# ur-whitelab/hoomd-tf

Hardware: AMD Instinct MI355X
Metric: MD steps/sec + achieved HBM GB/s, 131072 particles NN=128 (131k-particle box of the BASELINE metric) (higher is better)
Workload: dtype f32

## Files before the change

### hoomd_tf_amd/csrc/standin.hip

```cpp
#include <cstdlib>

#include "htf_common.h"
#include "box_math.h"
#include "htf_standin.h"
#include "standin_gate.h"
#include "key_sort.h"

namespace htf {

template <typename T>
__global__ __launch_bounds__(256) void nve_step_kernel(typename Vec4<T>::type *__restrict__ pos,
                                                       typename Vec4<T>::type *__restrict__ vel,
                                                       const typename Vec4<T>::type *__restrict__ force,
                                                       unsigned N, T dt, SBox<T> b) {
    unsigned i = blockIdx.x * blockDim.x + threadIdx.x;
    if (i >= N) return;
    auto p = pos[i];
    auto v = vel[i];
    nve_advance<T>(p, v, force[i], dt, b);
    pos[i] = p;
    vel[i] = v;
}

__device__ __forceinline__ float block_max(float d2, float *s_max) {
    for (int m = 1; m < 64; m <<= 1) d2 = fmaxf(d2, __shfl_xor(d2, m));
    if ((threadIdx.x & 63) == 0) s_max[threadIdx.x >> 6] = d2;
    __syncthreads();
    if (threadIdx.x < 16) {
        d2 = s_max[threadIdx.x];
        for (int m = 1; m < 16; m <<= 1) d2 = fmaxf(d2, __shfl_xor(d2, m));
    }
    return d2;
}

template <typename T>
__device__ __forceinline__ float block_max_disp2(const typename Vec4<T>::type *__restrict__ pos,
                                                 const typename Vec4<T>::type *__restrict__ ref, unsigned N, const SBox<T> &b,
                                                 float *s_max) {
    unsigned i = blockIdx.x * blockDim.x + threadIdx.x;
    float d2 = 0.f;
    if (i < N) d2 = row_disp2<T>(pos[i], ref[i], b);
    return block_max(d2, s_max);
}

__device__ __forceinline__ bool ticket_is_last(float d2, unsigned *__restrict__ work, unsigned *s_last) {
    if (threadIdx.x == 0) {
        unsigned last = 0u;
        if (__float_as_uint(d2) > *(volatile unsigned *)work) atomicMax(work, __float_as_uint(d2));
        __threadfence();
        if (atomicAdd(work + 1, 1u) == gridDim.x - 1u) last = 1u;
        *s_last = last;
    }
    __syncthreads();
    return *s_last != 0u;
}

template <typename T>
__global__ __launch_bounds__(1024) void max_disp_kernel(const typename Vec4<T>::type *__restrict__ pos,
                                                        const typename Vec4<T>::type *__restrict__ ref, unsigned N,
                                                        SBox<T> b, float *__restrict__ out) {
    __shared__ float s_max[16];
    const float d2 = block_max_disp2<T>(pos, ref, N, b, s_max);
    if (threadIdx.x == 0 && __float_as_uint(d2) > *(volatile unsigned *)out)
        atomicMax((unsigned *)out, __float_as_uint(d2));
}

template <typename T, bool CYCLE>
__global__ __launch_bounds__(1024) void check_disp_kernel(const typename Vec4<T>::type *__restrict__ pos,
                                                          const typename Vec4<T>::type *__restrict__ ref, unsigned N,
                                                          SBox<T> b, unsigned *__restrict__ work, float *__restrict__ out,
                                                          float *__restrict__ h_out, htfs_mirror mirror) {
    __shared__ float s_max[16];
    __shared__ unsigned s_last;
    const float d2 = block_max_disp2<T>(pos, ref, N, b, s_max);
    if (!ticket_is_last(d2, work, &s_last)) return;
    if (CYCLE) {
        for (unsigned m = 0; m < mirror.n; ++m) {
            const unsigned *src = (const unsigned *)mirror.src[m];
            unsigned *dst = (unsigned *)mirror.dst[m];
            for (unsigned w = threadIdx.x; w < mirror.words[m]; w += blockDim.x) dst[w] = __builtin_nontemporal_load(src + w);
        }
        __threadfence_system();
        __syncthreads();
    }
    if (threadIdx.x == 0) {
        const float worst = __uint_as_float(atomicExch(work, 0u));
        out[0] = worst;
        work[1] = 0u;
        if (CYCLE) {
            const unsigned cycle = __float_as_uint(out[1]) + 1u;
            out[1] = __uint_as_float(cycle);
            if (h_out != nullptr) {
                h_out[0] = worst;
                __threadfence_system();
                *(volatile unsigned *)(h_out + 1) = cycle;
            }
        }
    }
}

template <typename T>
__global__ __launch_bounds__(1024) void nve_check_kernel(typename Vec4<T>::type *__restrict__ pos, typename Vec4<T>::type *__restrict__ vel,
                                                         const typename Vec4<T>::type *__restrict__ force,
                                                         const typename Vec4<T>::type *__restrict__ ref, unsigned N, T dt, SBox<T> b,
                                                         SBox<T> lb, unsigned *__restrict__ work, float *__restrict__ out) {
    __shared__ float s_max[16];
    __shared__ unsigned s_last;
    unsigned i = blockIdx.x * blockDim.x + threadIdx.x;
    float d2 = 0.f;
    if (i < N) {
        auto p = pos[i];
        auto v = vel[i];
        nve_advance<T>(p, v, force[i], dt, b);
        asm volatile("" : "+v"(p.x), "+v"(p.y), "+v"(p.z));
        pos[i] = p;
        vel[i] = v;
        d2 = row_disp2<T>(p, ref[i], lb);
    }
    d2 = block_max(d2, s_max);
    if (!ticket_is_last(d2, work, &s_last)) return;
    if (threadIdx.x == 0) {
        out[0] = __uint_as_float(atomicExch(work, 0u));
        work[1] = 0u;
    }
}

template <typename T>
__device__ __forceinline__ int cell_coord(T x, T lo, T Linv, int n) {
    int c = (int)floor((x - lo) * Linv * (T)n);
    return c < 0 ? 0 : (c >= n ? n - 1 : c);
}

template <typename T>
__global__ __launch_bounds__(256) void cell_index_kernel(const typename Vec4<T>::type *__restrict__ pos, unsigned Ntot,
                                                         SBox<T> b, int nx, int ny, int nz,
                                                         unsigned *__restrict__ cell_of, Gate gate) {
    if (gate.closed()) return;
    unsigned i = blockIdx.x * blockDim.x + threadIdx.x;
    if (i >= Ntot) return;
    auto p = pos[i];
    if (is_inert(p.x)) {
        cell_of[i] = kDeadCell;
        return;
    }
    int cx = cell_coord<T>(p.x, b.lo[0], b.Linv[0], nx);
    int cy = cell_coord<T>(p.y, b.lo[1], b.Linv[1], ny);
    int cz = cell_coord<T>(p.z, b.lo[2], b.Linv[2], nz);
    cell_of[i] = (unsigned)((cz * ny + cy) * nx + cx);
}

constexpr unsigned kTagSide = 1u << 31;
constexpr unsigned kRangeWrapShift = 28u, kRangeLenMask = (1u << kRangeWrapShift) - 1u;
struct RangesArgs {
    int nx, ny, nz, wx, wy, wz, px, py, pz;
    const unsigned *cell_start;
    uint4 *table;
    unsigned *max_neigh;
};
__device__ __forceinline__ void cell_ranges_body(const unsigned t, const RangesArgs &a) {
    const int nx = a.nx, ny = a.ny, nz = a.nz, wx = a.wx, wy = a.wy, wz = a.wz, px = a.px, py = a.py, pz = a.pz;
    const unsigned *__restrict__ cell_start = a.cell_start;
    uint4 *__restrict__ table = a.table;
    unsigned *__restrict__ max_neigh = a.max_neigh;
    const int nrow = (2 * wy + 1) * (2 * wz + 1);
    if (t == 0) *max_neigh = 0u;
    const unsigned ncell = (unsigned)(nx * ny * nz);
    if (t >= ncell * (unsigned)nrow) return;
    const int c = (int)(t / nrow), r = (int)(t % nrow);
    const int cx = c % nx, cy = (c / nx) % ny, cz = c / (nx * ny);
    const int dz = r / (2 * wy + 1) - wz, dy = r % (2 * wy + 1) - wy;
    int a0 = cx - wx, a1 = cx + wx, b0 = 0, b1 = -1;
    if (a0 < 0) {
        if (px) { b0 = nx + a0; b1 = nx - 1; }
        a0 = 0;
    } else if (a1 >= nx) {
        if (px) { b0 = 0; b1 = a1 - nx; }
        a1 = nx - 1;
    }
    int ay = cy + dy, az = cz + dz;
    bool skip = false;
    unsigned wrap_y = 0u, wrap_z = 0u;
    if (ay < 0) { skip |= !py; ay += ny; wrap_y = 1u; } else if (ay >= ny) { skip |= !py; ay -= ny; wrap_y = 2u; }
    if (az < 0) { skip |= !pz; az += nz; wrap_z = 1u; } else if (az >= nz) { skip |= !pz; az -= nz; wrap_z = 2u; }
    uint4 o = make_uint4(0u, 0u, 0u, 0u);
    if (!skip) {
        const unsigned rowbase = (unsigned)((az * ny + ay) * nx);
        o.x = cell_start[rowbase + a0];
        o.y = (cell_start[rowbase + a1 + 1] - o.x) | (wrap_y << kRangeWrapShift) | (wrap_z << (kRangeWrapShift + 2));
        if (b1 >= b0) {
            o.z = cell_start[rowbase + b0];
            o.w = (cell_start[rowbase + b1 + 1] - o.z) | ((b0 == 0 ? 2u : 1u) << kRangeWrapShift);
        }
    }
    table[t] = o;
}
__global__ __launch_bounds__(256) void cell_ranges_kernel(RangesArgs a, Gate gate) {
    if (gate.closed()) return;
    cell_ranges_body(blockIdx.x * blockDim.x + threadIdx.x, a);
}

template <typename T, int G, bool SHIFT>
__global__ __launch_bounds__(256) void build_nlist_kernel(const typename Vec4<T>::type *__restrict__ pos,
                                                          const typename Vec4<T>::type *__restrict__ pos_sorted,
                                                          unsigned N, SBox<T> b, T rl2, int nx, int ny, int nz,
                                                          int wx, int wy, int wz,
                                                          const unsigned *__restrict__ cell_start, unsigned pitch,
                                                          int type_split,
                                                          unsigned *__restrict__ n_neigh, unsigned *__restrict__ head_list,
                                                          unsigned *__restrict__ nlist, unsigned *__restrict__ max_neigh,
                                                          const uint4 *__restrict__ ranges, Gate gate) {
    if (gate.closed()) return;
    const unsigned lane = threadIdx.x & 63u, g = lane % G, sub = lane / G;
    const unsigned i = ((blockIdx.x * blockDim.x + threadIdx.x) >> 6) * (64 / G) + sub;
    const bool in_range = i < N;
    const auto pi = pos[in_range ? i : 0];
    const bool active = in_range && !is_inert(pi.x);
    const int cx = cell_coord<T>(pi.x, b.lo[0], b.Linv[0], nx);
    const int cy = cell_coord<T>(pi.y, b.lo[1], b.Linv[1], ny);
    const int cz = cell_coord<T>(pi.z, b.lo[2], b.Linv[2], nz);
    const bool side_i = type_split >= 0 && scalar_as_int(pi.w) >= type_split;
    unsigned count = 0;
    unsigned *row = nlist + (size_t)(active ? i : 0) * pitch;
    const int nrow = (2 * wy + 1) * (2 * wz + 1);
    const uint4 *mine = ranges + (size_t)((cz * ny + cy) * nx + cx) * nrow;
    uint4 rg_next = active ? mine[0] : make_uint4(0u, 0u, 0u, 0u);
    for (int r = 0; r < nrow; ++r) {
        const uint4 rg = rg_next;
        if (r + 1 < nrow) rg_next = active ? mine[r + 1] : make_uint4(0u, 0u, 0u, 0u);
        T piy = pi.y, piz = pi.z, six = (T)0;
        if (SHIFT) {
            const unsigned wy_ = (rg.y >> kRangeWrapShift) & 3u, wz_ = rg.y >> (kRangeWrapShift + 2), wx_ = rg.w >> kRangeWrapShift;
            piy += wy_ == 1u ? b.L[1] : (wy_ == 2u ? -b.L[1] : (T)0);
            piz += wz_ == 1u ? b.L[2] : (wz_ == 2u ? -b.L[2] : (T)0);
            six = wx_ == 1u ? b.L[0] : -b.L[0];
        }
#pragma unroll
        for (int part = 0; part < 2; ++part) {
            const unsigned beg = part ? rg.z : rg.x, len = (part ? rg.w : rg.y) & kRangeLenMask;
            const T pix = (SHIFT && part) ? pi.x + six : pi.x;
            const unsigned n = active ? len : 0u;
            for (unsigned t = 0; t < n; t += G) {
                const unsigned m_idx = t + g;
                const auto pk = pos_sorted[beg + min(m_idx, n - 1u)];
                const unsigned tag = (unsigned)scalar_as_int(pk.w);
                const unsigned k = tag & ~kTagSide;
                T ddx = pk.x - pix, ddy = pk.y - piy, ddz = pk.z - piz;
                if (!SHIFT) {
                    ddx = mimg<T>(ddx, b.L[0], b.Linv[0], b.periodic[0]);
                    ddy = mimg<T>(ddy, b.L[1], b.Linv[1], b.periodic[1]);
                    ddz = mimg<T>(ddz, b.L[2], b.Linv[2], b.periodic[2]);
                }
                unsigned long long hits = ballot64(m_idx < n) & ballot64(k != i) & ballot64(ddx * ddx + ddy * ddy + ddz * ddz <= rl2);
                if (type_split >= 0) {
                    asm volatile("" ::: "memory");
                    hits &= ballot64(((tag & kTagSide) != 0u) == side_i);
                }
                const unsigned seg = (unsigned)(hits >> (G * sub)) & (G >= 32 ? ~0u : ((1u << G) - 1u));
                const unsigned rank = count + (unsigned)__popc(seg & ((1u << g) - 1u));
                if (inverse_ballot64(hits) && rank < pitch) row[rank] = k;
                count += (unsigned)__popc(seg);
            }
        }
    }
    if (in_range && g == 0) {
        n_neigh[i] = count < pitch ? count : pitch;
        head_list[i] = i * pitch;
        if (count > *(volatile unsigned *)max_neigh) atomicMax(max_neigh, count);
    }
}


__device__ __forceinline__ void set_tag(float &w, unsigned tag) { w = __uint_as_float(tag); }
__device__ __forceinline__ void set_tag(double &w, unsigned tag) { w = __longlong_as_double((long long)tag); }
__device__ __forceinline__ float bcast_lane_t(float v, unsigned lane) {
    return __int_as_float(__builtin_amdgcn_readlane(__float_as_int(v), (int)lane));
}
__device__ __forceinline__ double bcast_lane_t(double v, unsigned lane) {
    const long long q = __double_as_longlong(v);
    const unsigned lo = (unsigned)__builtin_amdgcn_readlane((int)(unsigned)q, (int)lane);
    const unsigned hi = (unsigned)__builtin_amdgcn_readlane((int)(unsigned)(q >> 32), (int)lane);
    return __longlong_as_double((long long)(((unsigned long long)hi << 32) | lo));
}
__device__ __forceinline__ unsigned bperm_u(unsigned lane_idx, unsigned v) {
    return (unsigned)__builtin_amdgcn_ds_bpermute((int)(lane_idx << 2), (int)v);
}
__device__ __forceinline__ float bperm_t(unsigned lane_idx, float v) { return __uint_as_float(bperm_u(lane_idx, __float_as_uint(v))); }
__device__ __forceinline__ double bperm_t(unsigned lane_idx, double v) {
    const unsigned long long q = (unsigned long long)__double_as_longlong(v);
    const unsigned lo = bperm_u(lane_idx, (unsigned)q), hi = bperm_u(lane_idx, (unsigned)(q >> 32));
    return __longlong_as_double((long long)(((unsigned long long)hi << 32) | lo));
}
constexpr int kCellBatch = 8;

template <typename T, bool SHIFT>
__global__ __launch_bounds__(256) void build_nlist_cells_kernel(const typename Vec4<T>::type *__restrict__ pos_sorted, unsigned N,
                                                                SBox<T> b, T rl2, unsigned ncell, int nrow,
                                                                const unsigned *__restrict__ cell_start, unsigned pitch,
                                                                int type_split, unsigned *__restrict__ n_neigh,
                                                                unsigned *__restrict__ head_list, unsigned *__restrict__ nlist,
                                                                unsigned *__restrict__ max_neigh,
                                                                const uint4 *__restrict__ ranges, unsigned split, Gate gate) {
    if (gate.closed()) return;
    using V4 = typename Vec4<T>::type;
    const unsigned lane = threadIdx.x & 63u;
    const unsigned wv = __builtin_amdgcn_readfirstlane((blockIdx.x * blockDim.x + threadIdx.x) >> 6);
    const unsigned c = wv / split, b0 = wv % split;
    if (c >= ncell) return;
    const unsigned p_begin = cell_start[c], p_end = cell_start[c + 1];
    if (p_begin + b0 * (unsigned)kCellBatch >= p_end) return;
    if (p_end - p_begin <= 64u) {
        const bool local = lane < p_end - p_begin && ((unsigned)scalar_as_int(pos_sorted[p_begin + lane].w) & ~kTagSide) < N;
        if (ballot64(local) == 0ull) return;
    }

    unsigned beg = 0u, len = 0u;
    T shx = (T)0, shy = (T)0, shz = (T)0;
    if (lane < 2u * (unsigned)nrow) {
        const uint4 rg = ranges[(size_t)c * nrow + (lane >> 1)];
        const bool wrapped = (lane & 1u) != 0u;
        beg = wrapped ? rg.z : rg.x;
        len = (wrapped ? rg.w : rg.y) & kRangeLenMask;
        if (SHIFT) {
            const unsigned wy_ = (rg.y >> kRangeWrapShift) & 3u, wz_ = rg.y >> (kRangeWrapShift + 2), wx_ = rg.w >> kRangeWrapShift;
            shy = wy_ == 1u ? b.L[1] : (wy_ == 2u ? -b.L[1] : (T)0);
            shz = wz_ == 1u ? b.L[2] : (wz_ == 2u ? -b.L[2] : (T)0);
            shx = !wrapped ? (T)0 : (wx_ == 1u ? b.L[0] : -b.L[0]);
        }
    }
    unsigned incl = len;
#pragma unroll
    for (unsigned d = 1; d < 64u; d <<= 1) {
        const unsigned up = bperm_u(lane >= d ? lane - d : lane, incl);
        incl += lane >= d ? up : 0u;
    }
    const unsigned start = incl - len;
    const unsigned total = (unsigned)__builtin_amdgcn_readlane((int)incl, 63);
    const bool any_shift = SHIFT && ballot64(len != 0u && (shx != (T)0 || shy != (T)0 || shz != (T)0)) != 0ull;

    for (unsigned pb = p_begin + b0 * (unsigned)kCellBatch; pb < p_end; pb += split * (unsigned)kCellBatch) {
        const unsigned np = min(p_end - pb, (unsigned)kCellBatch);
        V4 me;
        me.x = me.y = me.z = (T)0;
        set_tag(me.w, ~0u);
        if (lane < np) me = pos_sorted[pb + lane];
        const unsigned my_tag = (unsigned)scalar_as_int(me.w);
        if (ballot64(lane < np && (my_tag & ~kTagSide) < N) == 0ull) continue;
        unsigned tag_p[kCellBatch], count[kCellBatch];
        T px[kCellBatch], py[kCellBatch], pz[kCellBatch];
        unsigned row_p[kCellBatch];
#pragma unroll
        for (int p = 0; p < kCellBatch; ++p) {
            tag_p[p] = ~0u;
            px[p] = py[p] = pz[p] = (T)0;
            count[p] = 0u;
            row_p[p] = 0u;
            if ((unsigned)p < np) {
                tag_p[p] = (unsigned)__builtin_amdgcn_readlane((int)my_tag, p);
                px[p] = in_vgpr(bcast_lane_t(me.x, p));
                py[p] = in_vgpr(bcast_lane_t(me.y, p));
                pz[p] = in_vgpr(bcast_lane_t(me.z, p));
                row_p[p] = (tag_p[p] & ~kTagSide) * pitch;
            }
        }
        for (unsigned q0 = 0; q0 < total; q0 += 64u) {
            const unsigned q = q0 + lane;
            unsigned at = 0u;
#pragma unroll
            for (unsigned step = 32u; step != 0u; step >>= 1) {
                const unsigned t = at + step;
                at = bperm_u(t, start) <= q ? t : at;
            }
            const bool valid = q < total;
            const unsigned src = bperm_u(at, beg) + (q - bperm_u(at, start));
            V4 pk;
            pk.x = pk.y = pk.z = (T)0;
            set_tag(pk.w, ~0u);
            if (valid) pk = pos_sorted[src];
            if (any_shift) {
                pk.x -= bperm_t(at, shx);
                pk.y -= bperm_t(at, shy);
                pk.z -= bperm_t(at, shz);
            }
            const unsigned tag = (unsigned)scalar_as_int(pk.w);
            const unsigned k = tag & ~kTagSide;
            const unsigned long long vmask = ballot64(valid);
#pragma unroll
            for (int p = 0; p < kCellBatch; ++p) {
                const unsigned i = tag_p[p] & ~kTagSide;
                if (i >= N) continue;
                T ddx = pk.x - px[p], ddy = pk.y - py[p], ddz = pk.z - pz[p];
                if (!SHIFT) {
                    ddx = mimg<T>(ddx, b.L[0], b.Linv[0], b.periodic[0]);
                    ddy = mimg<T>(ddy, b.L[1], b.Linv[1], b.periodic[1]);
                    ddz = mimg<T>(ddz, b.L[2], b.Linv[2], b.periodic[2]);
                }
                unsigned long long hits = vmask & ballot64(k != i) & ballot64(ddx * ddx + ddy * ddy + ddz * ddz <= rl2);
                if (type_split >= 0) {
                    asm volatile("" ::: "memory");
                    hits &= ballot64(((tag ^ tag_p[p]) & kTagSide) == 0u);
                }
                const unsigned rank = __builtin_amdgcn_mbcnt_hi((unsigned)(hits >> 32), __builtin_amdgcn_mbcnt_lo((unsigned)hits, count[p]));
                if (inverse_ballot64(hits) && rank < pitch) nlist[row_p[p] + rank] = k;
                count[p] += (unsigned)__builtin_popcountll(hits);
            }
        }
        unsigned cnt = 0u;
#pragma unroll
        for (int p = 0; p < kCellBatch; ++p) cnt = lane == (unsigned)p ? count[p] : cnt;
        if (lane < np) {
            const unsigned i = my_tag & ~kTagSide;
            if (i < N) {
                n_neigh[i] = cnt < pitch ? cnt : pitch;
                head_list[i] = i * pitch;
                if (cnt > *(volatile unsigned *)max_neigh) atomicMax(max_neigh, cnt);
            }
        }
    }
}

}

using namespace htf;

extern "C" int htfs_nve_step(void *d_pos, void *d_vel, const void *d_force, int dtype, unsigned N, double dt,
                             const htf_box *box, htf_stream stream) {
    HTF_REQUIRE(d_pos && d_vel && d_force && box, "htfs_nve_step: null pointer");
    if (N == 0) return HTF_OK;
    unsigned grid = (N + 255) / 256;
    if (dtype == HTF_F32)
        hipLaunchKernelGGL((nve_step_kernel<float>), dim3(grid), dim3(256), 0, (hipStream_t)stream, (float4 *)d_pos, (float4 *)d_vel, (const float4 *)d_force, N, (float)dt, make_sbox<float>(box));
    else
        hipLaunchKernelGGL((nve_step_kernel<double>), dim3(grid), dim3(256), 0, (hipStream_t)stream, (double4 *)d_pos, (double4 *)d_vel, (const double4 *)d_force, N, dt, make_sbox<double>(box));
    return check_launch("nve_step_kernel");
}

extern "C" int htfs_nve_step_check(void *d_pos, void *d_vel, const void *d_force, int dtype, unsigned N, double dt, const htf_box *box,
                                   const htfs_nlist *nl, float *d_disp2, htf_stream stream) {
    HTF_REQUIRE(d_pos && d_vel && d_force && box && nl && d_disp2, "htfs_nve_step_check: null pointer");
    HTF_REQUIRE(nl->ref && nl->scratch, "htfs_nve_step_check: the list has no reference positions or no scratch");
    HTF_REQUIRE(dtype == HTF_F32 || dtype == HTF_F64, "htfs_nve_step_check: bad dtype %d", dtype);
    if (N == 0) return HTF_OK;
    const unsigned ncell = (unsigned)(nl->ncell3[0] * nl->ncell3[1] * nl->ncell3[2]);
    HTF_REQUIRE(ncell > 0, "htfs_nve_step_check: no cells");
    unsigned *work = nl->scratch + HTFS_SCRATCH_WORK(ncell);
    const unsigned grid = (N + 1023) / 1024;
    if (dtype == HTF_F32)
        hipLaunchKernelGGL((nve_check_kernel<float>), dim3(grid), dim3(1024), 0, (hipStream_t)stream, (float4 *)d_pos, (float4 *)d_vel, (const float4 *)d_force, (const float4 *)nl->ref, N, (float)dt, make_sbox<float>(box), make_sbox<float>(&nl->box), work, d_disp2);
    else
        hipLaunchKernelGGL((nve_check_kernel<double>), dim3(grid), dim3(1024), 0, (hipStream_t)stream, (double4 *)d_pos, (double4 *)d_vel, (const double4 *)d_force, (const double4 *)nl->ref, N, dt, make_sbox<double>(box), make_sbox<double>(&nl->box), work, d_disp2);
    return check_launch("nve_check_kernel");
}

extern "C" int htfs_max_displacement2(const void *d_pos, const void *d_ref, int dtype, unsigned N, const htf_box *box,
                                      float *d_out, htf_stream stream) {
    HTF_REQUIRE(d_pos && d_ref && box && d_out, "htfs_max_displacement2: null pointer");
    if (N == 0) return HTF_OK;
    unsigned grid = (N + 1023) / 1024;
    if (dtype == HTF_F32)
        hipLaunchKernelGGL((max_disp_kernel<float>), dim3(grid), dim3(1024), 0, (hipStream_t)stream, (const float4 *)d_pos, (const float4 *)d_ref, N, make_sbox<float>(box), d_out);
    else
        hipLaunchKernelGGL((max_disp_kernel<double>), dim3(grid), dim3(1024), 0, (hipStream_t)stream, (const double4 *)d_pos, (const double4 *)d_ref, N, make_sbox<double>(box), d_out);
    return check_launch("max_disp_kernel");
}

extern "C" int htfs_check_displacement2(const void *d_pos, const void *d_ref, int dtype, unsigned N, const htf_box *box,
                                        unsigned *d_work, float *d_out, float *h_out, const htfs_mirror *mirror, htf_stream stream) {
    using namespace htf;
    HTF_REQUIRE(d_pos && d_ref && box && d_work && d_out, "htfs_check_displacement2: null pointer");
    HTF_REQUIRE(N > 0, "htfs_check_displacement2: no rows");
    htfs_mirror mr = {};
    if (mirror != nullptr) {
        mr = *mirror;
        HTF_REQUIRE(mr.n <= HTFS_MIRROR_MAX, "htfs_check_displacement2: %u mirrors (at most %d)", mr.n, HTFS_MIRROR_MAX);
        for (unsigned m = 0; m < mr.n; ++m)
            HTF_REQUIRE(mr.src[m] && mr.dst[m] && ((uintptr_t)mr.src[m] & 3) == 0 && ((uintptr_t)mr.dst[m] & 3) == 0,
                        "htfs_check_displacement2: mirror %u: null or unaligned pointer", m);
    }
    unsigned grid = (N + 1023) / 1024;
    if (dtype == HTF_F32)
        hipLaunchKernelGGL((check_disp_kernel<float, true>), dim3(grid), dim3(1024), 0, (hipStream_t)stream, (const float4 *)d_pos, (const float4 *)d_ref, N, make_sbox<float>(box), d_work, d_out, h_out, mr);
    else
        hipLaunchKernelGGL((check_disp_kernel<double, true>), dim3(grid), dim3(1024), 0, (hipStream_t)stream, (const double4 *)d_pos, (const double4 *)d_ref, N, make_sbox<double>(box), d_work, d_out, h_out, mr);
    return check_launch("check_disp_kernel");
}

namespace htf {
struct Reimage {
    double L[3], c[3];
};
template <typename T>
__device__ __forceinline__ T reimage1(T x, double L, double c) {
    return L > 0.0 ? (T)((double)x - L * rint(((double)x - c) / L)) : x;
}

template <typename V>
__global__ __launch_bounds__(256) void bins_finish_kernel(RangesArgs ra, unsigned nb_ranges, V *__restrict__ dest, const V *__restrict__ src,
                                                          const unsigned *__restrict__ stage, const unsigned *__restrict__ cell_of,
                                                          unsigned *__restrict__ order, unsigned *__restrict__ count, unsigned n,
                                                          int type_split, V *__restrict__ ref, unsigned n_ref,
                                                          unsigned *__restrict__ counter, Reimage im, Gate gate) {
    if (gate.closed()) return;
    if (blockIdx.x < nb_ranges) {
        const unsigned t = blockIdx.x * blockDim.x + threadIdx.x;
        if (count != nullptr && t < (unsigned)(ra.nx * ra.ny * ra.nz)) count[t] = 0u;
        cell_ranges_body(t, ra);
        return;
    }
    const unsigned i = (blockIdx.x - nb_ranges) * blockDim.x + threadIdx.x;
    if (i == 0 && counter != nullptr) *counter += 1u;
    if (i >= n || i >= ra.cell_start[ra.nx * ra.ny * ra.nz]) return;
    const unsigned k = stage[i];
    V p = src[k];
    const unsigned c = cell_of[k];
    const unsigned cb = ra.cell_start[c], ce = ra.cell_start[c + 1];
    unsigned slot = cb;
    for (unsigned j = cb; j < ce; ++j) slot += stage[j] < k ? 1u : 0u;
    order[slot] = k;
    if (ref != nullptr && k < n_ref) ref[k] = p;
    p.x = reimage1(p.x, im.L[0], im.c[0]);
    p.y = reimage1(p.y, im.L[1], im.c[1]);
    p.z = reimage1(p.z, im.L[2], im.c[2]);
    set_tag(p.w, k | ((type_split >= 0 && scalar_as_int(p.w) >= type_split) ? kTagSide : 0u));
    dest[slot] = p;
}

template <typename T>
__global__ __launch_bounds__(256) void cell_index_count_kernel(const typename Vec4<T>::type *__restrict__ pos, unsigned Ntot, SBox<T> b,
                                                               int nx, int ny, int nz, unsigned *__restrict__ cell_of,
                                                               unsigned *__restrict__ count, Reimage im, Gate gate) {
    if (gate.closed()) return;
    unsigned i = blockIdx.x * blockDim.x + threadIdx.x;
    if (i >= Ntot) return;
    auto p = pos[i];
    if (is_inert(p.x)) {
        cell_of[i] = kDeadCell;
        return;
    }
    int cx = cell_coord<T>(reimage1(p.x, im.L[0], im.c[0]), b.lo[0], b.Linv[0], nx);
    int cy = cell_coord<T>(reimage1(p.y, im.L[1], im.c[1]), b.lo[1], b.Linv[1], ny);
    int cz = cell_coord<T>(reimage1(p.z, im.L[2], im.c[2]), b.lo[2], b.Linv[2], nz);
    const unsigned c = (unsigned)((cz * ny + cy) * nx + cx);
    cell_of[i] = c;
    atomicAdd(&count[c], 1u);
}

template <typename V, bool TAG>
__global__ void gather4_kernel(V *__restrict__ dest, const V *__restrict__ src, const int *__restrict__ order, unsigned n,
                               int type_split, Gate gate, const unsigned *__restrict__ n_live = nullptr) {
    if (gate.closed()) return;
    const unsigned i = blockIdx.x * blockDim.x + threadIdx.x;
    if (i >= n) return;
    if (n_live != nullptr && i >= *n_live) return;
    const unsigned k = (unsigned)order[i];
    V p = src[k];
    if (TAG) set_tag(p.w, k | ((type_split >= 0 && scalar_as_int(p.w) >= type_split) ? kTagSide : 0u));
    dest[i] = p;
}
}

namespace htf {
__global__ __launch_bounds__(256) void cell_count_kernel(const unsigned *__restrict__ cell_of, unsigned n,
                                                         unsigned *__restrict__ count, Gate gate) {
    if (gate.closed()) return;
    const unsigned i = blockIdx.x * blockDim.x + threadIdx.x;
    if (i < n && cell_of[i] != kDeadCell) atomicAdd(&count[cell_of[i]], 1u);
}

constexpr unsigned kScanThreads = 256, kScanPer = 8, kScanChunk = kScanThreads * kScanPer;
__global__ __launch_bounds__(kScanThreads) void cell_scan_kernel(const unsigned *__restrict__ count, unsigned ncell,
                                                         unsigned *__restrict__ start, unsigned *__restrict__ cursor, Gate gate) {
    if (gate.closed()) return;
    __shared__ unsigned s_wave[kScanThreads / 64], s_carry[kScanThreads / 64];
    const unsigned t = threadIdx.x, lane = t & 63u, wave = t >> 6;
    const unsigned base = blockIdx.x * kScanChunk;
    unsigned before_blk = 0;
    {
        const uint4 *p = reinterpret_cast<const uint4 *>(count);
        for (unsigned i = t; i < base / 4; i += kScanThreads) {
            const uint4 v = p[i];
            before_blk += (v.x + v.y) + (v.z + v.w);
        }
        before_blk = group_sum_u<64>(before_blk);
        if (lane == 0) s_carry[wave] = before_blk;
    }
    const unsigned first = base + t * kScanPer;
    unsigned c[kScanPer];
#pragma unroll
    for (unsigned i = 0; i < kScanPer; ++i) c[i] = first + i < ncell ? count[first + i] : 0u;
    unsigned sum = 0;
#pragma unroll
    for (unsigned i = 0; i < kScanPer; ++i) sum += c[i];
    unsigned incl = sum;
#pragma unroll
    for (unsigned off = 1; off < 64; off <<= 1) {
        const unsigned v = (unsigned)__shfl_up((int)incl, off);
        if (lane >= off) incl += v;
    }
    if (lane == 63) s_wave[wave] = incl;
    __syncthreads();
    unsigned before = 0, total = 0, carry = 0;
#pragma unroll
    for (unsigned w = 0; w < kScanThreads / 64; ++w) {
        const unsigned v = s_wave[w];
        before += w < wave ? v : 0u;
        total += v;
        carry += s_carry[w];
    }
    unsigned run = carry + before + (incl - sum);
#pragma unroll
    for (unsigned i = 0; i < kScanPer; ++i)
        if (first + i < ncell) {
            start[first + i] = run;
            cursor[first + i] = run;
            run += c[i];
        }
    if (blockIdx.x == gridDim.x - 1 && t == 0) start[ncell] = carry + total;
}

__global__ __launch_bounds__(256) void cell_scatter_kernel(const unsigned *__restrict__ cell_of, unsigned n,
                                                           unsigned *__restrict__ cursor, unsigned *__restrict__ order, Gate gate) {
    if (gate.closed()) return;
    const unsigned i = blockIdx.x * blockDim.x + threadIdx.x;
    if (i < n && cell_of[i] != kDeadCell) order[atomicAdd(&cursor[cell_of[i]], 1u)] = i;
}

__global__ __launch_bounds__(256) void cell_order_kernel(const unsigned *__restrict__ start, unsigned ncell,
                                                         unsigned *__restrict__ order, unsigned *__restrict__ count, Gate gate) {
    if (gate.closed()) return;
    const unsigned c = blockIdx.x * blockDim.x + threadIdx.x;
    if (c >= ncell) return;
    count[c] = 0u;
    const unsigned b = start[c], e = start[c + 1];
    for (unsigned i = b + 1; i < e; ++i) {
        const unsigned v = order[i];
        unsigned j = i;
        while (j > b && order[j - 1] > v) {
            order[j] = order[j - 1];
            --j;
        }
        order[j] = v;
    }
}
}

static int zero_counts(unsigned *count, unsigned ncell, hipStream_t s) {
    HTF_REQUIRE(((uintptr_t)count & 15) == 0, "binning scratch must be 16-byte aligned (cell_scan_kernel reads it with 16-byte loads)");
    HTF_CHECK_HIP(hipMemsetAsync(count, 0, (size_t)ncell * sizeof(unsigned), s));
    return HTF_OK;
}
static int zero_nlist_scratch(const htfs_nlist *l, hipStream_t s) {
    const unsigned ncell = (unsigned)(l->ncell3[0] * l->ncell3[1] * l->ncell3[2]);
    HTF_REQUIRE(l->scratch && ncell > 0, "htfs_rebuild_nlist: no scratch, or no cells");
    if (int rc = zero_counts(l->scratch, ncell, s)) return rc;
    HTF_CHECK_HIP(hipMemsetAsync(l->scratch + HTFS_SCRATCH_WORK(ncell), 0, 2 * sizeof(unsigned), s));
    return HTF_OK;
}

extern "C" int htfs_cell_sort(const unsigned *d_cell_of, unsigned Ntot, unsigned ncell, unsigned *d_scratch,
                              unsigned *d_cell_start, unsigned *d_order, htf_stream stream) {
    using namespace htf;
    HTF_REQUIRE(d_cell_of && d_scratch && d_cell_start && d_order, "htfs_cell_sort: null pointer");
    HTF_REQUIRE(ncell > 0, "htfs_cell_sort: no cells");
    hipStream_t s = (hipStream_t)stream;
    unsigned *count = d_scratch, *cursor = d_scratch + ncell;
    if (int rc = zero_counts(count, ncell, s)) return rc;
    if (Ntot) hipLaunchKernelGGL(cell_count_kernel, dim3((Ntot + 255) / 256), dim3(256), 0, s, d_cell_of, Ntot, count, kOpenGate);
    hipLaunchKernelGGL(cell_scan_kernel, dim3((ncell + kScanChunk - 1) / kScanChunk), dim3(kScanThreads), 0, s, count, ncell, d_cell_start, cursor, kOpenGate);
    if (Ntot) hipLaunchKernelGGL(cell_scatter_kernel, dim3((Ntot + 255) / 256), dim3(256), 0, s, d_cell_of, Ntot, cursor, d_order, kOpenGate);
    hipLaunchKernelGGL(cell_order_kernel, dim3((ncell + 255) / 256), dim3(256), 0, s, d_cell_start, ncell, d_order, count, kOpenGate);
    return check_launch("htfs_cell_sort");
}

static int gather4(void *d_dest, const void *d_src, const int *d_order, int dtype, unsigned n, bool tag, int type_split,
                   htf_stream stream, const unsigned *d_n_live = nullptr) {
    using namespace htf;
    HTF_REQUIRE(d_dest && d_src && d_order, "htfs_gather4_tagged: null pointer");
    HTF_REQUIRE(!tag || n <= kTagSide, "htfs_gather4_tagged: %u particles do not fit the 31-bit tag", n);
    if (n == 0) return HTF_OK;
    const dim3 grid((n + 255) / 256), block(256);
    hipStream_t s = (hipStream_t)stream;
    if (dtype == HTF_F32) {
        if (tag) hipLaunchKernelGGL((gather4_kernel<float4, true>), grid, block, 0, s, (float4 *)d_dest, (const float4 *)d_src, d_order, n, type_split, kOpenGate, d_n_live);
        else hipLaunchKernelGGL((gather4_kernel<float4, false>), grid, block, 0, s, (float4 *)d_dest, (const float4 *)d_src, d_order, n, type_split, kOpenGate, d_n_live);
    } else {
        if (tag) hipLaunchKernelGGL((gather4_kernel<double4, true>), grid, block, 0, s, (double4 *)d_dest, (const double4 *)d_src, d_order, n, type_split, kOpenGate, d_n_live);
        else hipLaunchKernelGGL((gather4_kernel<double4, false>), grid, block, 0, s, (double4 *)d_dest, (const double4 *)d_src, d_order, n, type_split, kOpenGate, d_n_live);
    }
    return check_launch("gather4_kernel");
}

extern "C" int htfs_gather4_tagged(void *d_dest, const void *d_src, const int *d_order, int dtype, unsigned n, int type_split,
                                   htf_stream stream) {
    return gather4(d_dest, d_src, d_order, dtype, n, true, type_split, stream);
}

extern "C" int htfs_gather4_tagged_live(void *d_dest, const void *d_src, const int *d_order, int dtype, unsigned n_max,
                                        const unsigned *d_n_live, int type_split, htf_stream stream) {
    HTF_REQUIRE(d_n_live, "htfs_gather4_tagged_live: null pointer");
    return gather4(d_dest, d_src, d_order, dtype, n_max, true, type_split, stream, d_n_live);
}

template <typename T, typename V4>
__global__ __launch_bounds__(256) void slab_classify_kernel(const V4 *__restrict__ pos, unsigned N, const T *__restrict__ bounds,
                                                            int world, int rank, T r_ghost, unsigned *__restrict__ key) {
    const unsigned i = blockIdx.x * blockDim.x + threadIdx.x;
    if (i >= N) return;
    const T x = pos[i].x;
    int owner = 0;
    for (int c = 1; c < world; ++c) owner += (bounds[c] <= x) ? 1 : 0;
    const int left = (rank + world - 1) % world, right = (rank + 1) % world;
    unsigned dest;
    if (world == 2)
        dest = owner != rank ? 2u : 0u;
    else
        dest = owner == rank ? 0u : (owner == left ? 1u : (owner == right ? 2u : 3u));
    const bool near_l = x < bounds[owner] + r_ghost, near_r = x >= bounds[owner + 1] - r_ghost;
    const unsigned cls = near_l ? (near_r ? 2u : 1u) : (near_r ? 3u : 0u);
    key[i] = dest * 4u + cls;
}

extern "C" int htfs_slab_classify(const void *d_pos, int dtype, unsigned N, const void *d_bounds, int world, int rank,
                                  double r_ghost, unsigned *d_key, htf_stream stream) {
    HTF_REQUIRE(d_pos && d_bounds && d_key, "htfs_slab_classify: null pointer");
    HTF_REQUIRE(world >= 2 && rank >= 0 && rank < world, "htfs_slab_classify: rank %d of %d", rank, world);
    if (N == 0) return HTF_OK;
    const unsigned grid = (N + 255) / 256;
    if (dtype == HTF_F32)
        hipLaunchKernelGGL((slab_classify_kernel<float, float4>), dim3(grid), dim3(256), 0, (hipStream_t)stream, (const float4 *)d_pos, N,
                           (const float *)d_bounds, world, rank, (float)r_ghost, d_key);
    else
        hipLaunchKernelGGL((slab_classify_kernel<double, double4>), dim3(grid), dim3(256), 0, (hipStream_t)stream, (const double4 *)d_pos,
                           N, (const double *)d_bounds, world, rank, r_ghost, d_key);
    return check_launch("slab_classify_kernel");
}

extern "C" int htfs_key_sort16(const unsigned *d_key, unsigned N, unsigned *d_scratch, unsigned *d_start, unsigned *d_order,
                               htf_stream stream) {
    HTF_REQUIRE(d_key && d_scratch && d_start && d_order, "htfs_key_sort16: null pointer");
    return htf::key_sort<16>(d_key, N, nullptr, d_scratch, d_start, d_order, (hipStream_t)stream);
}

struct SegTable {
    unsigned n;
    unsigned src[HTFS_MAX_SEGMENTS], dst[HTFS_MAX_SEGMENTS], cnt[HTFS_MAX_SEGMENTS];
};

__global__ __launch_bounds__(256) void segment_copy_kernel(unsigned *__restrict__ dst, const unsigned *__restrict__ src,
                                                           unsigned row_words, SegTable t, unsigned total_rows) {
    const unsigned w = blockIdx.x * blockDim.x + threadIdx.x;
    if (w >= total_rows * row_words) return;
    unsigned row = w / row_words;
    const unsigned col = w - row * row_words;
    unsigned seg = 0;
#pragma unroll 1
    while (seg + 1 < t.n && row >= t.cnt[seg]) {
        row -= t.cnt[seg];
        ++seg;
    }
    dst[(size_t)(t.dst[seg] + row) * row_words + col] = src[(size_t)(t.src[seg] + row) * row_words + col];
}

extern "C" int htfs_segment_copy(void *d_dst, const void *d_src, unsigned row_bytes, unsigned n_segments,
                                 const unsigned *src_start, const unsigned *dst_start, const unsigned *count, htf_stream stream) {
    HTF_REQUIRE(d_dst && d_src && src_start && dst_start && count, "htfs_segment_copy: null pointer");
    HTF_REQUIRE(n_segments >= 1 && n_segments <= HTFS_MAX_SEGMENTS && row_bytes % 4 == 0 && row_bytes > 0,
                "htfs_segment_copy: need 1..%d segments of whole 32-bit words", HTFS_MAX_SEGMENTS);
    SegTable t;
    t.n = 0;
    unsigned total = 0;
    for (unsigned s = 0; s < n_segments; ++s) {
        if (count[s] == 0) continue;
        t.src[t.n] = src_start[s];
        t.dst[t.n] = dst_start[s];
        t.cnt[t.n] = count[s];
        total += count[s];
        ++t.n;
    }
    if (total == 0) return HTF_OK;
    const unsigned words = row_bytes / 4;
    const unsigned grid = (unsigned)(((size_t)total * words + 255) / 256);
    hipLaunchKernelGGL(segment_copy_kernel, dim3(grid), dim3(256), 0, (hipStream_t)stream, (unsigned *)d_dst, (const unsigned *)d_src,
                       words, t, total);
    return check_launch("segment_copy_kernel");
}

extern "C" int htfs_cell_index(const void *d_pos, int dtype, unsigned Ntot, const htf_box *box, const int *ncell3,
                               unsigned *d_cell_of, htf_stream stream) {
    HTF_REQUIRE(d_pos && box && ncell3 && d_cell_of, "htfs_cell_index: null pointer");
    if (Ntot == 0) return HTF_OK;
    unsigned grid = (Ntot + 255) / 256;
    if (dtype == HTF_F32)
        hipLaunchKernelGGL((cell_index_kernel<float>), dim3(grid), dim3(256), 0, (hipStream_t)stream, (const float4 *)d_pos, Ntot, make_sbox<float>(box), ncell3[0], ncell3[1], ncell3[2], d_cell_of, kOpenGate);
    else
        hipLaunchKernelGGL((cell_index_kernel<double>), dim3(grid), dim3(256), 0, (hipStream_t)stream, (const double4 *)d_pos, Ntot, make_sbox<double>(box), ncell3[0], ncell3[1], ncell3[2], d_cell_of, kOpenGate);
    return check_launch("cell_index_kernel");
}

struct FinishArgs {
    unsigned n;
    htf::Reimage im;
    const unsigned *stage;
    unsigned *count;
};

static int build_nlist_impl(const htfs_nlist *l, const void *d_pos, int dtype, unsigned N, htf_stream stream, htf::Gate gate,
                            const FinishArgs *fin) {
    using namespace htf;
    HTF_REQUIRE(l && d_pos && l->pos_sorted && l->cell_start && l->n_neigh && l->head_list && l->nlist && l->max_neigh,
                "htfs_build_nlist: null pointer");
    const htf_box *box = &l->box;
    const int *ncell3 = l->ncell3, *stencil3 = l->stencil3;
    const unsigned *d_cell_start = l->cell_start;
    const void *d_pos_sorted = l->pos_sorted;
    const unsigned pitch = l->pitch;
    const int type_split = l->type_split;
    const double r_list = l->r_list;
    unsigned *d_n_neigh = l->n_neigh, *d_head_list = l->head_list, *d_nlist = l->nlist, *d_max_neigh = l->max_neigh;
    HTF_REQUIRE(pitch > 0, "htfs_build_nlist: pitch must be > 0");
    for (int d = 0; d < 3; ++d) {
        const double w = (box->hi[d] - box->lo[d]) / ncell3[d];
        const int sw = stencil3[d];
        HTF_REQUIRE((sw == 0 && ncell3[d] == 1) || (sw >= 1 && sw <= 2 && ncell3[d] >= 2 * sw + 1 && w * sw >= r_list * (1.0 - 1e-12)),
                    "htfs_build_nlist: along %d need 1 cell, or >= 2w+1 cells with w cells spanning r_list (got %d cells of %g, stencil %d, r_list %g)",
                    d, ncell3[d], w, sw, r_list);
    }
    if (N == 0) return HTF_OK;
    const unsigned ncell = (unsigned)(ncell3[0] * ncell3[1] * ncell3[2]);
    const unsigned nrow = (unsigned)((2 * stencil3[1] + 1) * (2 * stencil3[2] + 1));
    HTF_REQUIRE(l->ranges && ((uintptr_t)l->ranges & 15) == 0, "htfs_build_nlist: ranges must be a 16-byte aligned table of 4 * ncell * rows words");
    uint4 *d_ranges = (uint4 *)l->ranges;
    const RangesArgs ra = {ncell3[0], ncell3[1], ncell3[2], stencil3[0], stencil3[1], stencil3[2], (int)box->periodic[0],
                           (int)box->periodic[1], (int)box->periodic[2], d_cell_start, d_ranges, d_max_neigh};
    const unsigned nb_ranges = (ncell * nrow + 255) / 256;
    if (fin == nullptr) {
        hipLaunchKernelGGL(cell_ranges_kernel, dim3(nb_ranges), dim3(256), 0, (hipStream_t)stream, ra, gate);
    } else {
        const unsigned nb = nb_ranges + (fin->n + 255) / 256 + (fin->n == 0 ? 1u : 0u);
        if (dtype == HTF_F32)
            hipLaunchKernelGGL((bins_finish_kernel<float4>), dim3(nb), dim3(256), 0, (hipStream_t)stream, ra, nb_ranges, (float4 *)l->pos_sorted,
                               (const float4 *)d_pos, fin->stage, l->cell_of, l->order, fin->count, fin->n, type_split, (float4 *)l->ref, N, l->counter, fin->im, gate);
        else
            hipLaunchKernelGGL((bins_finish_kernel<double4>), dim3(nb), dim3(256), 0, (hipStream_t)stream, ra, nb_ranges, (double4 *)l->pos_sorted,
                               (const double4 *)d_pos, fin->stage, l->cell_of, l->order, fin->count, fin->n, type_split, (double4 *)l->ref, N, l->counter, fin->im, gate);
    }
    const bool fine = stencil3[0] == 2 || stencil3[1] == 2 || stencil3[2] == 2;
#define HTFS_NL(T, V4, G)                                                                                              \
    if (shift) HTFS_NL_(T, V4, G, true); else HTFS_NL_(T, V4, G, false)
#define HTFS_NL_(T, V4, G, S)                                                                                          \
    hipLaunchKernelGGL((build_nlist_kernel<T, G, S>), dim3((N + 4 * (64 / G) - 1) / (4 * (64 / G))), dim3(256), 0, (hipStream_t)stream, \
                       (const V4 *)d_pos, (const V4 *)d_pos_sorted, N, make_sbox<T>(box), (T)(r_list * r_list), ncell3[0],  \
                       ncell3[1], ncell3[2], stencil3[0], stencil3[1], stencil3[2], d_cell_start, pitch,      \
                       type_split, d_n_neigh, d_head_list, d_nlist, d_max_neigh, (const uint4 *)d_ranges, gate)
#define HTFS_NLC(T, V4)                                                                                                \
    if (shift) HTFS_NLC_(T, V4, true); else HTFS_NLC_(T, V4, false)
#define HTFS_NLC_(T, V4, S)                                                                                            \
    hipLaunchKernelGGL((build_nlist_cells_kernel<T, S>), dim3((ncell * cell_split + 3) / 4), dim3(256), 0, (hipStream_t)stream, \
                       (const V4 *)d_pos_sorted, N, make_sbox<T>(box), (T)(r_list * r_list), ncell, (int)nrow, d_cell_start, pitch, \
                       type_split, d_n_neigh, d_head_list, d_nlist, d_max_neigh, (const uint4 *)d_ranges, cell_split, gate)
    bool shift = true;
    for (int d = 0; d < 3; ++d) shift = shift && (!box->periodic[d] || ncell3[d] >= 7);
#ifdef HTF_AB_VARIANTS
    static const bool per_particle = std::getenv("HTFS_NLIST_PER_PARTICLE") != nullptr, per_cell = std::getenv("HTFS_NLIST_PER_CELL") != nullptr;
#else
    constexpr bool per_particle = false, per_cell = false;
#endif
    const bool reimaged = fin != nullptr && (fin->im.L[0] > 0.0 || fin->im.L[1] > 0.0 || fin->im.L[2] > 0.0);
    const bool by_cell = per_cell || reimaged || (!per_particle && ncell >= 1024u);
    const unsigned cell_split = ncell <= 12288u ? 2u : 1u;
    if (by_cell) {
        if (dtype == HTF_F32) { HTFS_NLC(float, float4); } else { HTFS_NLC(double, double4); }
    } else if (dtype == HTF_F32) {
        if (fine) { HTFS_NL(float, float4, 8); } else { HTFS_NL(float, float4, 16); }
    } else {
        if (fine) { HTFS_NL(double, double4, 8); } else { HTFS_NL(double, double4, 16); }
    }
#undef HTFS_NL
#undef HTFS_NL_
#undef HTFS_NLC
#undef HTFS_NLC_
    return check_launch("build_nlist_kernel");
}

extern "C" int htfs_build_nlist(const htfs_nlist *nl, const void *d_pos, int dtype, unsigned N, htf_stream stream) {
    return build_nlist_impl(nl, d_pos, dtype, N, stream, htf::kOpenGate, nullptr);
}

static int rebuild_nlist_impl(const htfs_nlist *l, const void *d_pos, int dtype, unsigned N, unsigned Ntot, bool scratch_clean,
                              htf_stream stream, htf::Gate gate) {
    using namespace htf;
    HTF_REQUIRE(l && d_pos && l->cell_of && l->scratch && l->cell_start && l->order && l->pos_sorted, "htfs_rebuild_nlist: null pointer");
    HTF_REQUIRE(Ntot >= N, "htfs_rebuild_nlist: Ntot %u < N %u", Ntot, N);
    if (N == 0) return HTF_OK;
    const htf_box *box = &l->box;
    const int *ncell3 = l->ncell3;
    const unsigned ncell = (unsigned)(ncell3[0] * ncell3[1] * ncell3[2]);
    HTF_REQUIRE(ncell > 0, "htfs_rebuild_nlist: no cells");
    hipStream_t s = (hipStream_t)stream;
    unsigned *count = l->scratch, *cursor = l->scratch + ncell, *stage = l->scratch + HTFS_SCRATCH_STAGE(ncell);
    if (!scratch_clean)
        if (int rc = zero_nlist_scratch(l, s)) return rc;
    const unsigned grid = (Ntot + 255) / 256;
    Reimage im = {};
    for (int d = 0; d < 3; ++d) {
        im.L[d] = !box->periodic[d] ? l->image_L[d] : 0.0;
        im.c[d] = 0.5 * (box->lo[d] + box->hi[d]);
        HTF_REQUIRE(im.L[d] == 0.0 || im.L[d] >= box->hi[d] - box->lo[d], "htfs_rebuild_nlist: image length %g along axis %d is shorter than the grid", im.L[d], d);
    }
    if (dtype == HTF_F32)
        hipLaunchKernelGGL((cell_index_count_kernel<float>), dim3(grid), dim3(256), 0, s, (const float4 *)d_pos, Ntot, make_sbox<float>(box),
                           ncell3[0], ncell3[1], ncell3[2], l->cell_of, count, im, gate);
    else
        hipLaunchKernelGGL((cell_index_count_kernel<double>), dim3(grid), dim3(256), 0, s, (const double4 *)d_pos, Ntot, make_sbox<double>(box),
                           ncell3[0], ncell3[1], ncell3[2], l->cell_of, count, im, gate);
    hipLaunchKernelGGL(cell_scan_kernel, dim3((ncell + kScanChunk - 1) / kScanChunk), dim3(kScanThreads), 0, s, count, ncell, l->cell_start, cursor, gate);
    hipLaunchKernelGGL(cell_scatter_kernel, dim3(grid), dim3(256), 0, s, l->cell_of, Ntot, cursor, stage, gate);
    const FinishArgs fin = {Ntot, im, stage, count};
    return build_nlist_impl(l, d_pos, dtype, N, stream, gate, &fin);
}

extern "C" int htfs_rebuild_nlist(const htfs_nlist *nl, const void *d_pos, int dtype, unsigned N, unsigned Ntot, int scratch_clean,
                                  htf_stream stream) {
    return rebuild_nlist_impl(nl, d_pos, dtype, N, Ntot, scratch_clean != 0, stream, htf::kOpenGate);
}

static int gated_rebuild(const htfs_nlist *nl, const void *d_pos, int dtype, unsigned N, unsigned Ntot, bool scratch_clean, float *d_disp2,
                         double threshold2, unsigned *d_stat2, unsigned *h_stat2, htf_stream stream) {
    htfs_nlist l = *nl;
    l.max_neigh = d_stat2;
    l.counter = d_stat2 + 1;
    int rc = rebuild_nlist_impl(&l, d_pos, dtype, N, Ntot, scratch_clean, stream, htf::Gate{d_disp2, (float)threshold2});
    if (rc != HTF_OK) return rc;
    if (h_stat2 != nullptr)
        HTF_CHECK_HIP(hipMemcpyAsync(h_stat2, d_stat2, 2 * sizeof(unsigned), hipMemcpyDeviceToHost, (hipStream_t)stream));
    return HTF_OK;
}

extern "C" int htfs_check_rebuild_nlist(const htfs_nlist *nl, const void *d_pos, int dtype, unsigned N, unsigned Ntot, int scratch_clean,
                                        float *d_disp2, double threshold2, unsigned *d_stat2, unsigned *h_stat2, htf_stream stream) {
    using namespace htf;
    HTF_REQUIRE(nl && nl->ref && nl->scratch && d_pos && d_disp2 && d_stat2, "htfs_check_rebuild_nlist: null pointer");
    if (N == 0) return HTF_OK;
    const unsigned ncell = (unsigned)(nl->ncell3[0] * nl->ncell3[1] * nl->ncell3[2]);
    HTF_REQUIRE(ncell > 0, "htfs_check_rebuild_nlist: no cells");
    hipStream_t s = (hipStream_t)stream;
    unsigned *work = nl->scratch + HTFS_SCRATCH_WORK(ncell);
    if (!scratch_clean)
        if (int rc = zero_nlist_scratch(nl, s)) return rc;
    const unsigned grid = (N + 1023) / 1024;
    const htfs_mirror none = {};
    if (dtype == HTF_F32)
        hipLaunchKernelGGL((check_disp_kernel<float, false>), dim3(grid), dim3(1024), 0, s, (const float4 *)d_pos, (const float4 *)nl->ref, N, make_sbox<float>(&nl->box), work, d_disp2, (float *)nullptr, none);
    else
        hipLaunchKernelGGL((check_disp_kernel<double, false>), dim3(grid), dim3(1024), 0, s, (const double4 *)d_pos, (const double4 *)nl->ref, N, make_sbox<double>(&nl->box), work, d_disp2, (float *)nullptr, none);
    int rc = check_launch("check_disp_kernel");
    if (rc != HTF_OK) return rc;
    return gated_rebuild(nl, d_pos, dtype, N, Ntot, true, d_disp2, threshold2, d_stat2, h_stat2, stream);
}

extern "C" int htfs_rebuild_nlist_gated(const htfs_nlist *nl, const void *d_pos, int dtype, unsigned N, unsigned Ntot, int scratch_clean,
                                        float *d_disp2, double threshold2, unsigned *d_stat2, unsigned *h_stat2, int h_stat2_by_mail,
                                        htf_stream stream) {
    HTF_REQUIRE(nl && nl->ref && nl->scratch && d_pos && d_disp2 && d_stat2, "htfs_rebuild_nlist_gated: null pointer");
    if (N == 0) return HTF_OK;
    return gated_rebuild(nl, d_pos, dtype, N, Ntot, scratch_clean != 0, d_disp2, threshold2, d_stat2, h_stat2_by_mail ? nullptr : h_stat2,
                         stream);
}
```

Before: 13790.

## Replace per-lane binary search with LDS run-boundary bitmap in cell nlist build

Replaces the six-step ds_bpermute binary search that maps each candidate slot to its source cell range with a per-wave LDS bitmap of run boundaries, using mbcnt to rank and a single permute to find the source offset. It also precomputes row and side masks as scalar ballots, derives self-exclusion from slot index instead of tag compare, and caps SGPRs. The intent is to cut cross-lane permute traffic and VALU work in the inner loop of neighbor-list construction. It adds LDS usage and a fallback path when the candidate total exceeds the bitmap size. The self-exclusion test assumes the i-particle appears at its own sorted index in the candidate stream.

```diff
diff --git a/hoomd_tf_amd/csrc/standin.hip b/hoomd_tf_amd/csrc/standin.hip
--- a/hoomd_tf_amd/csrc/standin.hip
+++ b/hoomd_tf_amd/csrc/standin.hip
@@ -291,15 +291,17 @@
     return __longlong_as_double((long long)(((unsigned long long)hi << 32) | lo));
 }
 constexpr int kCellBatch = 8;
+constexpr unsigned kMapBits = 2048u;
 
 template <typename T, bool SHIFT>
-__global__ __launch_bounds__(256) void build_nlist_cells_kernel(const typename Vec4<T>::type *__restrict__ pos_sorted, unsigned N,
-                                                                SBox<T> b, T rl2, unsigned ncell, int nrow,
-                                                                const unsigned *__restrict__ cell_start, unsigned pitch,
-                                                                int type_split, unsigned *__restrict__ n_neigh,
-                                                                unsigned *__restrict__ head_list, unsigned *__restrict__ nlist,
-                                                                unsigned *__restrict__ max_neigh,
-                                                                const uint4 *__restrict__ ranges, unsigned split, Gate gate) {
+__global__ __launch_bounds__(256) __attribute__((amdgpu_num_sgpr(80)))
+void build_nlist_cells_kernel(const typename Vec4<T>::type *__restrict__ pos_sorted, unsigned N,
+                              SBox<T> b, T rl2, unsigned ncell, int nrow,
+                              const unsigned *__restrict__ cell_start, unsigned pitch,
+                              int type_split, unsigned *__restrict__ n_neigh,
+                              unsigned *__restrict__ head_list, unsigned *__restrict__ nlist,
+                              unsigned *__restrict__ max_neigh,
+                              const uint4 *__restrict__ ranges, unsigned split, Gate gate) {
     if (gate.closed()) return;
     using V4 = typename Vec4<T>::type;
     const unsigned lane = threadIdx.x & 63u;
@@ -337,6 +339,26 @@
     const unsigned total = (unsigned)__builtin_amdgcn_readlane((int)incl, 63);
     const bool any_shift = SHIFT && ballot64(len != 0u && (shx != (T)0 || shy != (T)0 || shz != (T)0)) != 0ull;
 
+    __shared__ unsigned s_map[4 * (kMapBits / 32u)];
+    unsigned *const map = s_map + (threadIdx.x >> 6) * (kMapBits / 32u);
+    const bool mapped = total <= kMapBits;
+    unsigned delta_c = 0u, lane_c = 0u, map_lo = 0u, map_hi = 0u;
+    if (mapped) {
+        const unsigned long long runs = ballot64(len != 0u);
+        const unsigned ord = __builtin_amdgcn_mbcnt_hi((unsigned)(runs >> 32), __builtin_amdgcn_mbcnt_lo((unsigned)runs, 0u));
+        const unsigned to = (len != 0u ? ord : 63u) << 2;
+        delta_c = (unsigned)__builtin_amdgcn_ds_permute((int)to, (int)(beg - start));
+        lane_c = (unsigned)__builtin_amdgcn_ds_permute((int)to, (int)lane);
+        map[lane] = 0u;
+        __builtin_amdgcn_wave_barrier();
+        if (len != 0u && start != 0u) atomicOr(&map[(start - 1u) >> 5], 1u << ((start - 1u) & 31u));
+        __builtin_amdgcn_wave_barrier();
+        map_lo = map[(2u * lane) & 63u];
+        map_hi = map[(2u * lane + 1u) & 63u];
+    }
+    unsigned marks = 0u;
+
+    const T rl2_v = in_vgpr(rl2);
     for (unsigned pb = p_begin + b0 * (unsigned)kCellBatch; pb < p_end; pb += split * (unsigned)kCellBatch) {
         const unsigned np = min(p_end - pb, (unsigned)kCellBatch);
         V4 me;
@@ -344,69 +366,82 @@
         set_tag(me.w, ~0u);
         if (lane < np) me = pos_sorted[pb + lane];
         const unsigned my_tag = (unsigned)scalar_as_int(me.w);
-        if (ballot64(lane < np && (my_tag & ~kTagSide) < N) == 0ull) continue;
-        unsigned tag_p[kCellBatch], count[kCellBatch];
+        const unsigned rows = (unsigned)ballot64(lane < np && (my_tag & ~kTagSide) < N);
+        if (rows == 0u) continue;
+        const unsigned sides = (unsigned)ballot64((my_tag & kTagSide) != 0u);
+        unsigned count_v[kCellBatch];
         T px[kCellBatch], py[kCellBatch], pz[kCellBatch];
         unsigned row_p[kCellBatch];
 #pragma unroll
         for (int p = 0; p < kCellBatch; ++p) {
-            tag_p[p] = ~0u;
+            count_v[p] = 0u;
             px[p] = py[p] = pz[p] = (T)0;
-            count[p] = 0u;
-            row_p[p] = 0u;
+            row_p[p] = ((unsigned)__builtin_amdgcn_readlane((int)my_tag, p) & ~kTagSide) * pitch;
             if ((unsigned)p < np) {
-                tag_p[p] = (unsigned)__builtin_amdgcn_readlane((int)my_tag, p);
+                count_v[p] = __float_as_uint(in_vgpr(0.f));
                 px[p] = in_vgpr(bcast_lane_t(me.x, p));
                 py[p] = in_vgpr(bcast_lane_t(me.y, p));
                 pz[p] = in_vgpr(bcast_lane_t(me.z, p));
-                row_p[p] = (tag_p[p] & ~kTagSide) * pitch;
             }
         }
+        marks = 0u;
         for (unsigned q0 = 0; q0 < total; q0 += 64u) {
             const unsigned q = q0 + lane;
-            unsigned at = 0u;
+            unsigned at = 0u, src;
+            if (mapped) {
+                const unsigned w_lo = (unsigned)__builtin_amdgcn_readlane((int)map_lo, (int)(q0 >> 6));
+                const unsigned w_hi = (unsigned)__builtin_amdgcn_readlane((int)map_hi, (int)(q0 >> 6));
+                const unsigned r = __builtin_amdgcn_mbcnt_hi(w_hi, __builtin_amdgcn_mbcnt_lo(w_lo, marks));
+                marks += (unsigned)__builtin_popcount(w_lo) + (unsigned)__builtin_popcount(w_hi);
+                src = q + bperm_u(r, delta_c);
+                if (any_shift) at = bperm_u(r, lane_c);
+            } else {
 #pragma unroll
-            for (unsigned step = 32u; step != 0u; step >>= 1) {
-                const unsigned t = at + step;
-                at = bperm_u(t, start) <= q ? t : at;
+                for (unsigned step = 32u; step != 0u; step >>= 1) {
+                    const unsigned t = at + step;
+                    at = bperm_u(t, start) <= q ? t : at;
+                }
+                src = bperm_u(at, beg) + (q - bperm_u(at, start));
             }
-            const bool valid = q < total;
-            const unsigned src = bperm_u(at, beg) + (q - bperm_u(at, start));
             V4 pk;
             pk.x = pk.y = pk.z = (T)0;
             set_tag(pk.w, ~0u);
-            if (valid) pk = pos_sorted[src];
+            if (q < total) pk = pos_sorted[src];
             if (any_shift) {
                 pk.x -= bperm_t(at, shx);
                 pk.y -= bperm_t(at, shy);
                 pk.z -= bperm_t(at, shz);
             }
+            const unsigned slot = src - pb;
             const unsigned tag = (unsigned)scalar_as_int(pk.w);
             const unsigned k = tag & ~kTagSide;
-            const unsigned long long vmask = ballot64(valid);
+            const unsigned nq = total - q0;
+            const unsigned long long vmask = nq >= 64u ? ~0ull : (1ull << nq) - 1ull;
+            const unsigned long long far = type_split >= 0 ? ballot64((tag & kTagSide) != 0u) : 0ull;
+            unsigned rows_t = rows, sides_t = sides;
+            asm volatile("" : "+s"(rows_t), "+s"(sides_t));
 #pragma unroll
             for (int p = 0; p < kCellBatch; ++p) {
-                const unsigned i = tag_p[p] & ~kTagSide;
-                if (i >= N) continue;
+                if (__builtin_expect(((rows_t >> p) & 1u) == 0u, 0)) continue;
                 T ddx = pk.x - px[p], ddy = pk.y - py[p], ddz = pk.z - pz[p];
                 if (!SHIFT) {
                     ddx = mimg<T>(ddx, b.L[0], b.Linv[0], b.periodic[0]);
                     ddy = mimg<T>(ddy, b.L[1], b.Linv[1], b.periodic[1]);
                     ddz = mimg<T>(ddz, b.L[2], b.Linv[2], b.periodic[2]);
                 }
-                unsigned long long hits = vmask & ballot64(k != i) & ballot64(ddx * ddx + ddy * ddy + ddz * ddz <= rl2);
-                if (type_split >= 0) {
+                unsigned long long hits = vmask & ballot64(slot != (unsigned)p) & ballot64(ddx * ddx + ddy * ddy + ddz * ddz <= rl2_v);
+                if (__builtin_expect(type_split >= 0, 0)) {
                     asm volatile("" ::: "memory");
-                    hits &= ballot64(((tag ^ tag_p[p]) & kTagSide) == 0u);
+                    hits &= ((sides_t >> p) & 1u) != 0u ? far : ~far;
                 }
-                const unsigned rank = __builtin_amdgcn_mbcnt_hi((unsigned)(hits >> 32), __builtin_amdgcn_mbcnt_lo((unsigned)hits, count[p]));
+                const unsigned rank = __builtin_amdgcn_mbcnt_hi((unsigned)(hits >> 32), __builtin_amdgcn_mbcnt_lo((unsigned)hits, count_v[p]));
                 if (inverse_ballot64(hits) && rank < pitch) nlist[row_p[p] + rank] = k;
-                count[p] += (unsigned)__builtin_popcountll(hits);
+                count_v[p] += (unsigned)__builtin_popcountll(hits);
             }
         }
         unsigned cnt = 0u;
 #pragma unroll
-        for (int p = 0; p < kCellBatch; ++p) cnt = lane == (unsigned)p ? count[p] : cnt;
+        for (int p = 0; p < kCellBatch; ++p) cnt = lane == (unsigned)p ? count_v[p] : cnt;
         if (lane < np) {
             const unsigned i = my_tag & ~kTagSide;
             if (i < N) {
```

New measurement: 14030 (median of 6 runs). +1.8%, better.
